# pangenome/gfasort

Hardware: AMD Instinct MI355X
Metric: SGD term-updates/sec, -p Y, 1M-node synthetic GFA (higher is better)
Workload: dtype f64

## Files before the change

gfasort_amd/build.py:

```python
import os
import subprocess
import sys

HERE = os.path.dirname(os.path.abspath(__file__))
CSRC = os.path.join(HERE, "csrc")
LIBDIR = os.path.join(HERE, "lib")
LIB = os.path.join(LIBDIR, "libgfasort_hip.so")
SOURCES = ["sgd_kernels_1d.hip", "sgd_kernels_1d_phased.hip", "sgd_kernels_nd.hip", "sgd_kernels_nd_team.hip", "sgd_kernels_nd_team_wide.hip", "index_kernels.hip",
           "capi.hip", "multi.hip"]
HEADERS = ["sgd_device.h", "sgd_kernel_common.h", "sgd_1d.h", "sgd_nd_team.h", "sgd_host.h", os.path.join("..", "..", "include", "gfasort_hip.h")]

HIPCC_FLAGS = ["--offload-arch=gfx950", "-O3", "-std=c++17", "-fPIC",
               "-ffp-contract=off", "-munsafe-fp-atomics", "-Wall", "-Wno-unused-function"]
OBJDIR = os.path.join(HERE, "lib", "obj")


def _stale():
    if not os.path.exists(LIB):
        return True
    t = os.path.getmtime(LIB)
    deps = [os.path.join(CSRC, s) for s in SOURCES + HEADERS] + [os.path.abspath(__file__)]
    return any(os.path.getmtime(d) > t for d in deps)


def build_hip(force=False, verbose=False):
    if not force and not _stale():
        return LIB
    os.makedirs(OBJDIR, exist_ok=True)
    hipcc = os.environ.get("HIPCC", "/opt/rocm/bin/hipcc")
    hdr_t = max(os.path.getmtime(os.path.join(CSRC, h)) for h in HEADERS)

    def compile_one(src):
        obj = os.path.join(OBJDIR, src.replace(".hip", ".o"))
        sp = os.path.join(CSRC, src)
        if not force and os.path.exists(obj) and os.path.getmtime(obj) > max(os.path.getmtime(sp), hdr_t):
            return obj
        cmd = [hipcc] + HIPCC_FLAGS + ["-c", "-o", obj, sp]
        if verbose:
            print(" ".join(cmd), file=sys.stderr)
        subprocess.check_call(cmd)
        return obj

    from concurrent.futures import ThreadPoolExecutor
# ... 48 lines not shown
```

gfasort_amd/csrc/sgd_1d.h:

```cpp
#pragma once
#include "sgd_kernel_common.h"

namespace gfs {

struct RefTerm1D { uint32_t i, j; int crowd; double term_dist; };

template <bool LDS_TABLES>
__device__ __forceinline__ bool ref_sample_1d(const KArgs &a, const uint4 *path_tab, const double *zeta_tab, Rng &rng,
                                              const uint64_t step_idx, const uint4 &ra, RefTerm1D &t) {
    uint4 rb; uint64_t sa, sb; uint32_t cnt, path;
    if (!sample_pair_from<LDS_TABLES>(a, path_tab, zeta_tab, rng, step_idx, ra, rb, sa, sb, cnt, path)) return false;
    t.term_dist = fabs(rec_pos(ra) - rec_pos(rb));
    if (t.term_dist == 0.0) return false;
    t.crowd = crowd_shift<false>(a, ra, rb);
    t.i = ra.x; t.j = rb.x;
    return t.i != 0xFFFFFFFFu && t.j != 0xFFFFFFFFu;
}

template <bool LDS_TABLES, bool ATOMIC_LOADS, bool TRACE>
__device__ __forceinline__ void ref_run_1d(const KArgs &a, const uint4 *path_tab, const double *zeta_tab, Rng &rng,
                                           const uint32_t quota, const uint64_t max_att, const uint32_t tid,
                                           uint32_t &done, uint32_t &att, uint32_t &ntr) {
    double *x = a.x;
    uint32_t d = 0; uint64_t t = 0;
// ... 5 lines not shown
        RefTerm1D cur;
        if (!ref_sample_1d<LDS_TABLES>(a, path_tab, zeta_tab, rng, s_a, r_a, cur)) continue;
        const double mu = crowd_scale(fmin(a.it.eta * (1.0 / cur.term_dist), 1.0), cur.crowd);
        double dx;
        if (a.dbg & 2u) dx = (double)cur.i - (double)cur.j;
        else dx = load_pos<ATOMIC_LOADS>(x + cur.i) - load_pos<ATOMIC_LOADS>(x + cur.j);
        if (dx == 0.0) dx = 1e-9;
        const double mag = fabs(dx);
        const double delta = mu * (mag - cur.term_dist) / 2.0;
        const double r = delta / mag;
        const double r_x = r * dx;
        if (d + 1u < quota && t < max_att) { s_a = sample_step(a, rng); r_a = a.step_rec[s_a]; drawn = true; }
        if (a.dbg & 1u) { asm volatile("" :: "v"(r_x)); }
        else {
            add_pos(x + cur.i, -r_x);
            add_pos(x + cur.j, r_x);
        }
        ++d;
        if (TRACE) record_trace(a, tid, ntr, cur.i, cur.j, cur.term_dist);
    }
    done += d;
    att += t > 0xFFFFFFFFull ? 0xFFFFFFFFu : (uint32_t)t;
}

struct TeamState {
    Rng rng;
    Leader L = {0, 0, 0, 0, 0, 0, 0, 0};
    uint32_t left = 0, cool = 0, colour = 0, seg = 0;
    uint32_t p = 0;
    uint32_t done = 0, att = 0, ntr = 0;
};

struct Trip {
    uint64_t sa = 0, sb = 0;
    uint4 ra = make_uint4(0, 0, 0, 0), rb = make_uint4(0, 0, 0, 0);
    uint4 rc = make_uint4(0, 0, 0, 0);
    bool twin = false;
    bool valid = false;
    int mshift = 0;
    bool two = false;
    bool fused = false;
    uint32_t k = 1;
    uint32_t off = 0;
};

template <int B>
__device__ __forceinline__ void expand_trip(const KArgs &a, const Leader &L, int t, uint32_t seg, uint32_t p, uint32_t colour, int sub, int q, Trip &tr) {
    constexpr int RUNS = 64 / B;
    const int ll = t * RUNS + q;
    const uint32_t okw = bcast<B>(L.ok, ll), cnt = bcast<B>(L.cnt, ll);
    const uint32_t ok = leader_ok(okw, p);
    const uint32_t ra0 = p ? bcast<B>(L.ra1, ll) : bcast<B>(L.ra0, ll), rb0 = p ? bcast<B>(L.rb1, ll) : bcast<B>(L.rb0, ll);
    const uint64_t first = bcast_first<B>(L, ll);
    tr.k = (B == 64 && ((okw | (okw >> 8)) & 1u) && cnt >= 2u * B) ? run_trips(a.chain, (uint32_t)B, cnt) : 1u;
    tr.off = B == 64 ? run_offset((uint32_t)B, cnt, tr.k, ra0, rb0, seg) : 0u;
    tr.mshift = merged_trip_shift<B>(ok, cnt, ra0, rb0, tr.off);
    const bool two = !(a.dbg & 0x08u) && two_colour<B>(ok, cnt, ra0, rb0);
    tr.two = B == 64 ? two : (__any(two) != 0);
    tr.ra = make_uint4(0, 0, 0, 0); tr.rb = make_uint4(0, 0, 0, 0); tr.rc = make_uint4(0, 0, 0, 0);
    tr.fused = B == 64 && tr.mshift != 0 && colour == 0 && two && !(a.dbg & 0x100u);
    tr.twin = B == 64 && p == 0u && a.partners == 2u && (okw & 3u) == 3u && ((okw >> 8) & 3u) == 3u && !(a.dbg & 0x04u);
    const uint32_t rb1 = bcast<B>(L.rb1, ll);
    if (tr.twin) {
        const int64_t gap = (int64_t)rb0 - (int64_t)rb1, lim = 192;
        if (gap < lim && gap > -lim) tr.twin = false;
    }
    if (tr.twin) {
        tr.sa = first + ra0 + tr.off + (uint32_t)sub;
        tr.sb = first + rb0 + tr.off + (((uint32_t)sub + ((okw >> 2) & 7u)) & 63u);
        const uint64_t sc = first + rb1 + tr.off + (((uint32_t)sub + ((okw >> 10) & 7u)) & 63u);
        tr.valid = true;
        tr.ra = a.step_rec[tr.sa]; tr.rb = a.step_rec[tr.sb]; tr.rc = a.step_rec[sc];
        return;
    }
    if (tr.fused) {
        const int dst = sub + tr.mshift;
        tr.sa = first + merged_trip_base(cnt, ra0, tr.off) + (uint32_t)sub;
        tr.sb = (uint64_t)((int64_t)tr.sa + tr.mshift);
        tr.valid = dst < 0 || dst > 63;
        tr.ra = a.step_rec[tr.sa];
        tr.rb = a.step_rec[tr.sb];
        return;
    }
    tr.valid = expand_run<B>(ok, first, cnt, ra0, rb0, sub, colour, tr.off, tr.sa, tr.sb);
    if (tr.valid) { tr.ra = a.step_rec[tr.sa]; tr.rb = a.step_rec[tr.sb]; }
}

__device__ __forceinline__ double term_move(const KArgs &a, double term_dist, double xi, double xj, int crowd) {
    double mu = crowd_scale(fmin(a.it.eta * (1.0 / term_dist), 1.0), crowd);
    double dx = xi - xj;
    if (dx == 0.0) dx = 1e-9;
    double mag = fabs(dx);
    double delta = mu * (mag - term_dist) / 2.0;
    double r = delta / mag;
    return r * dx;
}

__device__ __forceinline__ double shfl_f64(double v, int src) { return __shfl(v, src, 64); }

template <bool ATOMIC_LOADS, bool TRACE>
__device__ __forceinline__ bool fused_trip(const KArgs &a, TeamState &ts, const Trip &cur, const int lane,
                                           const uint32_t tid, const uint64_t wave_quota, uint64_t &wave_done) {
    double *x = a.x;
    const int s = cur.mshift, z = s < 0 ? -s : s;
    const int dst = lane + s, src = lane - s;
    const bool out = cur.valid;
    const int dstc = out ? lane : dst, srcc = (src < 0 || src > 63) ? lane : src;
    const uint32_t grp = ((cur.off + (uint32_t)lane) / (uint32_t)z) & 1u;
    const uint32_t node = cur.ra.x, pnode = cur.rb.x;
    double xo = 0.0, xp = 0.0;
    if (!(a.dbg & 2u)) {
        if (node != 0xFFFFFFFFu) xo = load_pos<ATOMIC_LOADS>(x + node);
        if (out && pnode != 0xFFFFFFFFu) xp = load_pos<ATOMIC_LOADS>(x + pnode);
    } else { xo = (double)node; xp = (double)pnode; }
    const double term_dist = fabs(rec_pos(cur.ra) - rec_pos(cur.rb));
    const int crowd = crowd_shift<true>(a, cur.ra, cur.rb);
    const bool term_ok = term_dist != 0.0 && node != 0xFFFFFFFFu && pnode != 0xFFFFFFFFu;
    double acc = 0.0;
    bool touched = false, second = true;
#pragma unroll
    for (uint32_t colour = 0; colour < 2u; ++colour) {
        ++ts.att;
        const bool valid = quota_cut(term_ok && grp == colour, lane, wave_quota, wave_done);
        const double xpart_in = shfl_f64(xo, dstc);
        const double xj = out ? xp : xpart_in;
        double r_x = 0.0;
        if (valid) {
            r_x = term_move(a, term_dist, xo, xj, crowd);
            ++ts.done;
            if (TRACE) record_trace(a, tid, ts.ntr, node, pnode, term_dist);
        }
        const double rv = shfl_f64(r_x, srcc);
        const int vsrc = __shfl((int)valid, srcc, 64);
        const bool recv = src >= 0 && src <= 63 && vsrc != 0;
        if (valid) xo = xo - r_x;
        if (recv) xo = xo + rv;
        if (valid) { acc = touched ? acc - r_x : -r_x; touched = true; }
        if (recv) { acc = touched ? acc + rv : rv; touched = true; }
        if (valid && out && !(a.dbg & 1u)) add_pos(x + pnode, r_x);
        if (colour == 0 && wave_done >= wave_quota) { second = false; break; }
    }
    if (touched && !(a.dbg & 1u)) add_pos(x + node, acc);
    return second;
}

template <bool ATOMIC_LOADS, bool TRACE>
__device__ __forceinline__ bool twin_trip(const KArgs &a, TeamState &ts, const Trip &cur, const int lane,
                                          const uint32_t tid, const uint64_t wave_quota, uint64_t &wave_done) {
    double *x = a.x;
    const uint32_t node = cur.ra.x, nb = cur.rb.x, nc = cur.rc.x;
    double xa = 0.0, xb = 0.0, xc = 0.0;
    if (!(a.dbg & 2u)) {
        if (node != 0xFFFFFFFFu) xa = load_pos<ATOMIC_LOADS>(x + node);
        if (nb != 0xFFFFFFFFu) xb = load_pos<ATOMIC_LOADS>(x + nb);
        if (nc != 0xFFFFFFFFu) xc = load_pos<ATOMIC_LOADS>(x + nc);
    } else { xa = (double)node; xb = (double)nb; xc = (double)nc; }
    const double pa = rec_pos(cur.ra);
    double acc = 0.0;
    bool touched = false, second = true;
#pragma unroll
    for (uint32_t p = 0; p < 2u; ++p) {
        ++ts.att;
        const uint4 &rp = p ? cur.rc : cur.rb;
        const uint32_t pn = p ? nc : nb;
        const double term_dist = fabs(pa - rec_pos(rp));
        const bool valid = quota_cut(term_dist != 0.0 && node != 0xFFFFFFFFu && pn != 0xFFFFFFFFu,
                                     lane, wave_quota, wave_done);
        if (valid) {
            const double r_x = term_move(a, term_dist, xa, p ? xc : xb, crowd_shift<true>(a, cur.ra, rp));
            ++ts.done;
            if (TRACE) record_trace(a, tid, ts.ntr, node, pn, term_dist);
            xa = xa - r_x;
            acc = touched ? acc - r_x : -r_x; touched = true;
            if (!(a.dbg & 1u)) add_pos(x + pn, r_x);
        }
        if (p == 0u && wave_done >= wave_quota) { second = false; break; }
    }
    if (touched && !(a.dbg & 1u)) add_pos(x + node, acc);
    return second;
}

template <int B, bool LDS_TABLES, bool ATOMIC_LOADS, bool TRACE>
__device__ __forceinline__ void team_iteration(const KArgs &a, const uint4 *path_tab, const double *zeta_tab,
                                               TeamState &ts, const uint32_t tid, const uint64_t wave_quota, const IterConsts *itp = nullptr) {
    const int lane = threadIdx.x & 63;
    const int sub = lane & (B - 1);
    const int q = lane / B;
    const uint64_t max_passes = (uint64_t)a.attempt_factor * (wave_quota / (64u * B) + 1u) + 16u;
    uint64_t wave_done = 0, passes = 0;
    double *x = a.x;
    while (wave_done < wave_quota && passes < max_passes) {
        if (ts.left == 0 || ts.cool != (uint32_t)a.it.cooling) {
            ++passes;
            KArgs as;
            reload_kargs(as);
            if (itp) {
                const IterConsts *ip = itp;
                asm volatile("" : "+s"(ip));
                as.it = *ip;
            }
            ts.L = sample_leader<LDS_TABLES>(as, path_tab, zeta_tab, ts.rng);
            ts.left = B; ts.cool = (uint32_t)a.it.cooling; ts.colour = 0; ts.seg = 0; ts.p = 0;
        }
        const Leader &L = ts.L;
        int t = B - (int)ts.left;
        uint32_t colour = ts.colour, seg = ts.seg, p = ts.p;
        Trip cur;
        expand_trip<B>(a, L, t, seg, p, colour, sub, q, cur);
        for (;;) {
            int t_n = t; uint32_t colour_n = 0u, seg_n = seg, p_n = p;
            if (colour == 0 && cur.two && !cur.fused) colour_n = 1u;
            else if (p == 0u && a.partners == 2u && !cur.twin) p_n = 1u;
            else if (seg + 1u < cur.k) { seg_n = seg + 1u; p_n = 0u; }
            else { t_n = t + 1; seg_n = 0u; p_n = 0u; }
            const bool have_n = t_n < B;
            Trip nxt;
            if (have_n) expand_trip<B>(a, L, t_n, seg_n, p_n, colour_n, sub, q, nxt);
            if (B == 64 && cur.twin) {
                if (!twin_trip<ATOMIC_LOADS, TRACE>(a, ts, cur, lane, tid, wave_quota, wave_done)) {
                    ts.colour = 0u; ts.seg = seg; ts.p = 1u;
                    break;
                }
                ts.colour = 0u; ts.seg = seg_n; ts.p = 0u;
                if (t_n != t) --ts.left;
                if (wave_done >= wave_quota || !have_n) break;
                cur = nxt; t = t_n; colour = colour_n; seg = seg_n; p = p_n;
                continue;
            }
            if (B == 64 && cur.fused) {
                if (!fused_trip<ATOMIC_LOADS, TRACE>(a, ts, cur, lane, tid, wave_quota, wave_done)) {
                    ts.colour = 1u; ts.seg = seg; ts.p = p;
                    break;
                }
                ts.colour = 0u; ts.seg = seg_n; ts.p = p_n;
                if (t_n != t) --ts.left;
                if (wave_done >= wave_quota || !have_n) break;
                cur = nxt; t = t_n; colour = colour_n; seg = seg_n; p = p_n;
                continue;
            }
            ++ts.att;
            ts.colour = colour_n; ts.seg = seg_n; ts.p = p_n;
            if (t_n != t) --ts.left;
            bool valid = cur.valid;
            const uint4 ra = cur.ra, rb = cur.rb;
            const int mshift = cur.mshift;
            double term_dist = 0.0;
            uint32_t i = 0, j = 0;
            if (valid) {
                term_dist = fabs(rec_pos(ra) - rec_pos(rb));
                i = ra.x; j = rb.x;
                valid = term_dist != 0.0 && i != 0xFFFFFFFFu && j != 0xFFFFFFFFu;
            }
            valid = quota_cut(valid, lane, wave_quota, wave_done);
            double xi = 0.0, xj = 0.0;
            if (valid) {
                if (a.dbg & 2u) { xi = (double)i; xj = (double)j; }
                else { xi = load_pos<ATOMIC_LOADS>(x + i); xj = load_pos<ATOMIC_LOADS>(x + j); }
            }
            double r_x = 0.0;
            if (valid) {
                r_x = term_move(a, term_dist, xi, xj, crowd_shift<true>(a, ra, rb));
                ++ts.done;
                if (TRACE) record_trace(a, tid, ts.ntr, i, j, term_dist);
            }
            bool o1f = valid, o2f = valid; uint32_t o1s = i, o2s = j; double o1v = -r_x, o2v = r_x;
            if (B == 64 && mshift != 0) {
                const int z = mshift < 0 ? -mshift : mshift;
                const int src = lane - mshift;
                const int srcc = src < 0 ? 0 : (src > 63 ? 63 : src);
                const double rv = __shfl(r_x, srcc, 64);
                const uint32_t js = (uint32_t)__shfl((int)j, srcc, 64);
                const int vs = __shfl((int)valid, srcc, 64);
                const bool resting = (((cur.off + (uint32_t)lane) / (uint32_t)z) & 1u) != colour;
                if (resting && src >= 0 && src < 64 && vs) { o1f = true; o1s = js; o1v = rv; }
                const int dst = lane + mshift;
                o2f = valid && (dst < 0 || dst > 63);
            }
            if (!(a.dbg & 1u)) {
                if (o1f) add_pos(x + o1s, o1v);
                if (o2f) add_pos(x + o2s, o2v);
            }
            if (wave_done >= wave_quota) break;
            if (!have_n) break;
            cur = nxt; t = t_n; colour = colour_n; seg = seg_n; p = p_n;
        }
    }
// ... 4 lines not shown
```

gfasort_amd/csrc/sgd_device.h:

```cpp
#pragma once
#include <hip/hip_runtime.h>
#include <stdint.h>

namespace gfs {

__device__ __forceinline__ int32_t sat_i32(double v) {
    if (v != v) return 0;
    if (v <= -2147483648.0) return INT32_MIN;
    if (v >= 2147483647.0) return INT32_MAX;
    return (int32_t)v;
}

__device__ __forceinline__ double fpp_split(double a, int32_t e, double fb) {
    int32_t high = (int32_t)((uint64_t)__double_as_longlong(a) >> 32);
    int32_t diff = (int32_t)((uint32_t)high - 1072632447u);
    int32_t new_high = sat_i32(fb * (double)diff + 1072632447.0);
    double frac = __longlong_as_double((long long)(((uint64_t)(uint32_t)new_high) << 32));
    double base = a, r = 1.0;
    int32_t ex = e;
    while (ex != 0) {
        if (ex & 1) r *= base;
        base *= base;
        ex >>= 1;
    }
    return r * frac;
}

struct Rng {
    uint64_t s0, s1, s2, s3;
    __device__ __forceinline__ uint64_t next() {
        uint64_t result = s0 + s3;
        uint64_t t = s1 << 17;
        s2 ^= s0; s3 ^= s1; s1 ^= s2; s0 ^= s3;
        s2 ^= t;
        s3 = (s3 << 45) | (s3 >> 19);
// ... 121 lines not shown
        if (back || fwd) {
            uint32_t room = back ? rank_a : (cnt - rank_a - 1u);
            uint32_t jump = a.space < room ? a.space : room;
            double zeta = zeta_tab[space_index(a, jump)];
            uint32_t z = dirty_zipf(a.it, jump, zeta, rng.f64());
            if (back) rank_b = rank_a >= z ? rank_a - z : 0u;
            else { uint64_t t = (uint64_t)rank_a + z; rank_b = t < cnt - 1u ? (uint32_t)t : cnt - 1u; }
        }
    } else {
        rank_b = rng.uniform32(cnt, pr.z);
    }
    if (rank_a == rank_b) return false;
    sa = step_idx;
    sb = first + rank_b;
    rb = a.step_rec[sb];
    cnt_out = cnt; path_out = path;
    return true;
}
template <bool LDS_TABLES>
__device__ __forceinline__ bool sample_pair(const KArgs &a, const uint4 *path_tab, const double *zeta_tab,
                                            Rng &rng, uint4 &ra, uint4 &rb, uint64_t &sa, uint64_t &sb,
                                            uint32_t &cnt_out, uint32_t &path_out) {
    const uint64_t step_idx = sample_step(a, rng);
    ra = a.step_rec[step_idx];
    return sample_pair_from<LDS_TABLES>(a, path_tab, zeta_tab, rng, step_idx, ra, rb, sa, sb, cnt_out, path_out);
}

struct Leader {
    uint32_t first_lo, first_hi, cnt;
    uint32_t ra0, rb0;
    uint32_t ok;
    uint32_t ra1, rb1;
};
__device__ __forceinline__ uint32_t leader_ok(uint32_t okw, uint32_t p) { return (p ? okw >> 8 : okw) & 0x1Fu; }

constexpr uint32_t TEAM_CHUNK = 2048;
constexpr uint32_t ND_TEAM_CHUNK = 4096;

__device__ __forceinline__ uint32_t run_trips(uint32_t chain, uint32_t bundle, uint32_t cnt) {
    const uint32_t room = cnt / (4u * bundle);
    if (room < 2u || chain < 2u) return 1u;
    const uint32_t p2 = 1u << (31 - __clz((int)room));
    return p2 < chain ? p2 : chain;
}
__device__ __forceinline__ uint32_t run_offset(uint32_t bundle, uint32_t cnt, uint32_t k, uint32_t ra0, uint32_t rb0, uint32_t seg) {
    const uint32_t z = ra0 < rb0 ? rb0 - ra0 : ra0 - rb0;
    return seg * (z < bundle ? cnt / k : bundle);
}

__device__ __forceinline__ uint32_t draw_partner(const KArgs &a, const double *zeta_tab, Rng &rng, const uint32_t cnt,
                                                 const uint32_t thresh, const uint32_t slot0, uint32_t &ra, uint32_t &rb) {
    rb = ra;
    if (a.it.cooling || rng.flip() == 1u) {
        bool back = false, fwd = false;
        if (ra > 0u && (rng.flip() == 1u || ra == cnt - 1u)) back = true;
        else if (ra < cnt - 1u) fwd = true;
        if (back || fwd) {
            uint32_t room = back ? ra : (cnt - ra - 1u);
            uint32_t jump = a.space < room ? a.space : room;
            double zeta = zeta_tab[space_index(a, jump)];
            uint32_t z = dirty_zipf(a.it, jump, zeta, rng.f64());
            if (back) rb = ra >= z ? ra - z : 0u;
            else { uint64_t t = (uint64_t)ra + z; rb = t < cnt - 1u ? (uint32_t)t : cnt - 1u; }
        }
    } else {
        rb = rng.uniform32(cnt, thresh);
    }
    uint32_t ok = (rb != ra) ? 1u : 0u;
    if (ok && cnt >= 2u * a.bundle && slot0 != 0xFFFFFFFFu && !(a.dbg & 0x10u)) {
        const int64_t jump = (int64_t)rb - (int64_t)ra;
        const int64_t Bn = (int64_t)a.bundle;
        const int64_t Rn = Bn * (int64_t)run_trips(a.chain, a.bundle, cnt);
        if (jump >= Bn + 8 || jump <= -(Bn + 8)) {
            const int64_t A = a.bundle < 8u ? (int64_t)a.bundle : 8;
            const uint32_t sh = slot0 & (uint32_t)(A - 1);
            if (ra >= sh) {
                const int64_t na = (int64_t)ra - (int64_t)sh;
                const int64_t r = ((jump % A) + A) % A, zp = jump - r, nb = na + zp;
                if (!(a.dbg & 0x20u) && na + Rn <= (int64_t)cnt && nb >= 0 && nb + Rn <= (int64_t)cnt && (zp >= Bn || zp <= -Bn)) {
                    ra = (uint32_t)na; rb = (uint32_t)nb; ok = 1u | 2u | ((uint32_t)r << 2);
                } else if (rb >= sh) { ra -= sh; rb -= sh; }
            }
        }
    }
    return ok;
}

template <bool LDS_TABLES>
__device__ __forceinline__ Leader sample_leader(const KArgs &a, const uint4 *path_tab, const double *zeta_tab, Rng &rng) {
    Leader L;
    const uint64_t s0 = sample_step(a, rng);
    const uint4 r0 = a.step_rec[s0];
    const uint4 pr = path_tab[rec_path(r0)];
    L.first_lo = pr.x; L.first_hi = pr.w; L.cnt = pr.y;
    L.ra0 = (uint32_t)(s0 - path_first(pr)); L.rb0 = L.ra0;
    L.ra1 = L.ra0; L.rb1 = L.ra0;
    L.ok = 0;
    if (L.cnt == 1u) return L;
    L.ok = draw_partner(a, zeta_tab, rng, L.cnt, pr.z, r0.x, L.ra0, L.rb0);
    if (a.partners == 2u) L.ok |= draw_partner(a, zeta_tab, rng, L.cnt, pr.z, r0.x, L.ra1, L.rb1) << 8;
    return L;
}

template <int B>
__device__ __forceinline__ bool two_colour(uint32_t ok, uint32_t cnt, uint32_t ra0, uint32_t rb0) {
    if ((ok & 3u) != 1u || cnt < 2u * B) return false;
    const int64_t s = (int64_t)rb0 - (int64_t)ra0;
    return s < (int64_t)B && s > -(int64_t)B;
}

template <int B>
__device__ __forceinline__ bool expand_run(uint32_t ok, uint64_t first, uint32_t cnt, uint32_t ra0, uint32_t rb0,
                                           int sub, uint32_t colour, uint32_t off, uint64_t &sa, uint64_t &sb) {
    if (!(ok & 1u)) return false;
    if (ok & 2u) {
        if (colour) return false;
        sa = first + ra0 + off + (uint32_t)sub;
        sb = first + rb0 + off + (((uint32_t)sub + ((ok >> 2) & 7u)) & (uint32_t)(B - 1));
        return true;
    }
    uint32_t ra_l = ra0, rb_l = rb0;
    const uint32_t l = off + (uint32_t)sub;
    if (l != 0 || colour) {
        if (cnt < 2u * B) return false;
        const int64_t shift = (int64_t)rb0 - (int64_t)ra0;
        const uint32_t z = (uint32_t)(shift < 0 ? -shift : shift);
        if (z < (uint32_t)B) { if (((l / z) & 1u) != colour) return false; }
        else if (colour) return false;
        uint64_t ra_w = (uint64_t)ra0 + l;
        if (ra_w >= cnt) ra_w -= cnt;
        if (ra_w >= cnt) ra_w -= cnt;
        ra_l = (uint32_t)ra_w;
        int64_t t = (int64_t)ra_l + shift;
        if (t < 0 || t > (int64_t)cnt - 1) {
            if (z < (uint32_t)B) return false;
            t = (int64_t)ra_l - shift;
            if (t < 0 || t > (int64_t)cnt - 1) return false;
        }
        rb_l = (uint32_t)t;
    }
    sa = first + ra_l;
    sb = first + rb_l;
    return true;
}

__device__ __forceinline__ double rec_pos(const uint4 &r) {
    return (double)rec_pos_u64(r);
}

}
```

gfasort_amd/csrc/sgd_kernel_common.h:

```cpp
#pragma once
#include "sgd_device.h"

namespace gfs {

struct TraceTerm { uint32_t i, j; double d; };

template <bool ATOMIC_LOADS>
__device__ __forceinline__ double load_pos(const double *p) {
    if (ATOMIC_LOADS)
        return __hip_atomic_load(p, __ATOMIC_RELAXED, __HIP_MEMORY_SCOPE_AGENT);
    return *p;
}
__device__ __forceinline__ void add_pos(double *p, double v) {
    (void)__hip_atomic_fetch_add(p, v, __ATOMIC_RELAXED, __HIP_MEMORY_SCOPE_AGENT);
}

template <bool LDS_TABLES>
__device__ __forceinline__ void stage_tables(const KArgs &a, unsigned char *smem,
                                             const uint4 *&path_tab, const double *&zeta_tab) {
    if (LDS_TABLES) {
        uint4 *lp = reinterpret_cast<uint4 *>(smem);
        double *lz = reinterpret_cast<double *>(smem + (size_t)a.n_paths * sizeof(uint4));
        for (uint32_t k = threadIdx.x; k < a.n_paths; k += blockDim.x) lp[k] = a.path_rec[k];
        for (uint32_t k = threadIdx.x; k < a.zlen_staged; k += blockDim.x) lz[k] = a.zetas[k];
// ... 80 lines not shown
    return (uint32_t)__shfl((int)v, leader_lane, 64);
}


template <int B>
__device__ __forceinline__ uint64_t bcast_first(const Leader &L, int leader_lane) {
    return ((uint64_t)bcast<B>(L.first_hi, leader_lane) << 32) | bcast<B>(L.first_lo, leader_lane);
}

template <class State>
__device__ __forceinline__ void load_pass(const KArgs &a, uint32_t tid, State &ts, uint32_t &flips) {
    if (!a.lead) return;
    const uint64_t T = a.n_streams;
    ts.L.first_lo = a.lead[tid]; ts.L.first_hi = a.lead[T + tid]; ts.L.cnt = a.lead[2 * T + tid];
    ts.L.ra0 = a.lead[3 * T + tid]; ts.L.rb0 = a.lead[4 * T + tid];
    const uint32_t w = a.lead[5 * T + tid];
    ts.L.ra1 = a.lead[6 * T + tid]; ts.L.rb1 = a.lead[7 * T + tid];
    ts.L.ok = (w & 0x1Fu) | ((w >> 27) << 8);
    flips = (w >> 5) & 7u;
    const uint32_t ws = (uint32_t)__builtin_amdgcn_readfirstlane((int)w);
    ts.left = (ws >> 8) & 0xFFu; ts.cool = (ws >> 16) & 1u; ts.colour = (ws >> 17) & 1u; ts.seg = (ws >> 18) & 0xFFu; ts.p = (ws >> 26) & 1u;
}
template <class State>
__device__ __forceinline__ void store_pass(const KArgs &a, uint32_t tid, const State &ts, const uint32_t flips) {
    if (!a.lead) return;
    const uint64_t T = a.n_streams;
    a.lead[tid] = ts.L.first_lo; a.lead[T + tid] = ts.L.first_hi; a.lead[2 * T + tid] = ts.L.cnt;
    a.lead[3 * T + tid] = ts.L.ra0; a.lead[4 * T + tid] = ts.L.rb0;
    a.lead[5 * T + tid] = (ts.L.ok & 0x1Fu) | ((flips & 7u) << 5) | (ts.left << 8) | (ts.cool << 16) | (ts.colour << 17) | (ts.seg << 18) |
                          (ts.p << 26) | (((ts.L.ok >> 8) & 0x1Fu) << 27);
    a.lead[6 * T + tid] = ts.L.ra1; a.lead[7 * T + tid] = ts.L.rb1;
}

template <int B>
__device__ __forceinline__ int merged_trip_shift(uint32_t ok, uint32_t cnt, uint32_t ra0, uint32_t rb0, uint32_t off) {
    if (B != 64 || (ok & 3u) != 1u || cnt < 128u) return 0;
    const int64_t s = (int64_t)rb0 - (int64_t)ra0;
    if (s == 0 || s >= 64 || s <= -64) return 0;
    uint64_t base = (uint64_t)ra0 + (uint64_t)off;
    if (base >= cnt) base -= cnt;
    if (base + 64u > cnt) return 0;
    if (s > 0 ? base + 63u + (uint64_t)s > (uint64_t)cnt - 1u : (int64_t)base + s < 0) return 0;
    return (int)s;
}
__device__ __forceinline__ uint32_t merged_trip_base(uint32_t cnt, uint32_t ra0, uint32_t off) {
    uint64_t base = (uint64_t)ra0 + (uint64_t)off;
    if (base >= cnt) base -= cnt;
    return (uint32_t)base;
}

constexpr uint32_t POOL_SLOTS = 16, POOL_STRIDE = 16;
__host__ __device__ __forceinline__ uint32_t pool_slots(uint32_t n_waves) {
    const uint32_t s = n_waves / 16u;
    return s < 1u ? 1u : (s > POOL_SLOTS ? POOL_SLOTS : s);
}

struct PoolShare { uint32_t slot, cap; };
__device__ __forceinline__ PoolShare pool_share(const KArgs &a, const uint32_t wave, const uint32_t n_waves) {
    const uint32_t slots = pool_slots(n_waves), slot = wave % slots;
    const uint64_t total = (uint64_t)a.quota_base * a.n_streams + a.quota_rem;
    return {slot, (uint32_t)(total / slots + (slot < total % slots ? 1u : 0u))};
}
__device__ __forceinline__ PoolShare pool_share_single(const KArgs &a) {
    return {0u, (uint32_t)((uint64_t)a.quota_base * a.n_streams + a.quota_rem)};
}

__device__ __forceinline__ void send_claim(uint32_t *pool_counter, const uint32_t chunk, uint32_t &claim) {
    if ((threadIdx.x & 63u) == 0) claim = __hip_atomic_fetch_add(pool_counter, chunk, __ATOMIC_RELAXED, __HIP_MEMORY_SCOPE_AGENT);
}

template <class ChunkOf, class Body>
__device__ __forceinline__ void pool_walk(KArgs &a, const IterConsts *its, const uint32_t n_iters, uint32_t *pool, const PoolShare ps,
                                          ChunkOf &&chunk_of, Body &&body) {
    uint32_t k = 0, claim = 0;
    a.it = its[0];
    uint32_t chunk = chunk_of();
    send_claim(pool + ps.slot * POOL_STRIDE, chunk, claim);
    while (k < n_iters) {
        const uint32_t old = (uint32_t)__builtin_amdgcn_readfirstlane((int)claim);
        if (old >= ps.cap) {
            if (++k == n_iters) break;
            a.it = its[k];
// ... 27 lines not shown
```

Baseline: 104.5 billion.

## Hoist per-slot trip planning out of per-trip expansion and add fast quota path

Leader-slot fields (k, short jumps, twin flag, ok bits) are now computed once per slot into a packed SlotPlan instead of being re-broadcast and recomputed for every trip expansion. Step addresses are split into a wave-uniform base plus a small per-lane offset, which may let the compiler use scalar base addressing. A cheaper quota_cut_1d counts valid lanes with a ballot popcount when the remaining wave quota is at least 64. The shared helpers move into a host/device header with a host selftest that checks equivalence against the old logic. The cost is extra live registers for the plan, which could lower occupancy.

```diff
diff --git a/gfasort_amd/build.py b/gfasort_amd/build.py
--- a/gfasort_amd/build.py
+++ b/gfasort_amd/build.py
@@ -8,7 +8,7 @@
 LIB = os.path.join(LIBDIR, "libgfasort_hip.so")
 SOURCES = ["sgd_kernels_1d.hip", "sgd_kernels_1d_phased.hip", "sgd_kernels_nd.hip", "sgd_kernels_nd_team.hip", "sgd_kernels_nd_team_wide.hip", "index_kernels.hip",
            "capi.hip", "multi.hip"]
-HEADERS = ["sgd_device.h", "sgd_kernel_common.h", "sgd_1d.h", "sgd_nd_team.h", "sgd_host.h", os.path.join("..", "..", "include", "gfasort_hip.h")]
+HEADERS = ["sgd_device.h", "sgd_trip_plan.h", "sgd_kernel_common.h", "sgd_1d.h", "sgd_nd_team.h", "sgd_host.h", os.path.join("..", "..", "include", "gfasort_hip.h")]
 
 HIPCC_FLAGS = ["--offload-arch=gfx950", "-O3", "-std=c++17", "-fPIC",
                "-ffp-contract=off", "-munsafe-fp-atomics", "-Wall", "-Wno-unused-function"]
diff --git a/gfasort_amd/csrc/host/trip_plan_selftest.cpp b/gfasort_amd/csrc/host/trip_plan_selftest.cpp
--- /dev/null
+++ b/gfasort_amd/csrc/host/trip_plan_selftest.cpp
@@ -0,0 +1,126 @@
+#include <cinttypes>
+#include <cstdio>
+#include <cstdlib>
+#include <vector>
+#include "../sgd_trip_plan.h"
+
+using namespace gfs;
+
+static unsigned long long n_plans = 0, n_trips = 0, n_lanes = 0;
+
+#define CHECK(cond)                                                                                                           \
+    do {                                                                                                                      \
+        if (!(cond)) {                                                                                                        \
+            std::printf("DIFF %s (line %d): cnt %u chain %u okw 0x%x ra0 %u rb0 %u ra1 %u rb1 %u seg %u p %u colour %u sub %d dbg 0x%x partners %u\n", \
+                        #cond, __LINE__, cnt, chain, okw, ra0, rb0, ra1, rb1, seg, p, colour, sub, dbg, partners);            \
+            std::exit(1);                                                                                                     \
+        }                                                                                                                     \
+    } while (0)
+
+template <int B>
+static void sweep_leader(uint32_t chain, uint32_t partners, uint32_t dbg, uint64_t first, uint32_t cnt, uint32_t okw,
+                         uint32_t ra0, uint32_t rb0, uint32_t ra1, uint32_t rb1, uint32_t meta_rep, bool deep, int lane_step) {
+    uint32_t seg = 0, p = 0, colour = 0; int sub = 0;
+    const SlotPlan pl = make_plan<B>(chain, partners, dbg, first, cnt, okw, ra0, rb0, ra1, rb1);
+    ++n_plans;
+    const uint32_t k_old = (B == 64 && ((okw | (okw >> 8)) & 1u) && cnt >= 2u * B) ? run_trips(chain, (uint32_t)B, cnt) : 1u;
+    CHECK(pl.k() == k_old && pl.okw() == okw && pl.first == first && pl.cnt == cnt && pl.spread == cnt / k_old);
+    bool twin_old = B == 64 && partners == 2u && (okw & 3u) == 3u && ((okw >> 8) & 3u) == 3u && !(dbg & 0x04u);
+    if (twin_old) { const int64_t gap = (int64_t)rb0 - (int64_t)rb1, lim = 192; if (gap < lim && gap > -lim) twin_old = false; }
+    CHECK(pl.twin() == twin_old);
+    if (!deep) { CHECK(pl.meta == meta_rep); return; }
+    for (seg = 0; seg < k_old; ++seg) for (p = 0; p < partners; ++p) for (colour = 0; colour < 2u; ++colour) {
+        const uint32_t ok = leader_ok(okw, p), ra = p ? ra1 : ra0, rb = p ? rb1 : rb0;
+        const uint32_t off_old = B == 64 ? run_offset((uint32_t)B, cnt, k_old, ra, rb, seg) : 0u;
+        const int mshift_old = merged_trip_shift<B>(ok, cnt, ra, rb, off_old);
+        const bool two_old = !(dbg & 0x08u) && two_colour<B>(ok, cnt, ra, rb);
+        const bool fused_old = B == 64 && mshift_old != 0 && colour == 0 && two_old && !(dbg & 0x100u);
+        const bool twin_trip_old = p == 0u && twin_old;
+        if (colour == 1u && !two_old) continue;
+        const TripShape s = plan_trip<B>(pl, dbg, seg, p, colour);
+        ++n_trips;
+        CHECK(s.off == off_old);
+        CHECK(s.mshift == mshift_old && s.two == two_old && s.fused == fused_old && s.twin == twin_trip_old);
+        if (mshift_old != 0) CHECK(s.base == merged_trip_base(cnt, ra, off_old));
+        for (sub = 0; sub < B; sub += lane_step) {
+            LaneSteps ls;
+            const bool loads = trip_lane_steps<B>(pl, s, p, colour, sub, ls);
+            ++n_lanes;
+            if (twin_trip_old) {
+                CHECK(loads && ls.base_a + ls.la == first + ra0 + off_old + (uint32_t)sub);
+                CHECK(ls.base_b + ls.lb == first + rb0 + off_old + (((uint32_t)sub + ((okw >> 2) & 7u)) & 63u));
+                CHECK(ls.base_c + ls.lc == first + rb1 + off_old + (((uint32_t)sub + ((okw >> 10) & 7u)) & 63u));
+            } else if (fused_old) {
+                const uint64_t sa = first + merged_trip_base(cnt, ra, off_old) + (uint32_t)sub;
+                CHECK(loads && ls.base_a + ls.la == sa && ls.base_b + ls.lb == (uint64_t)((int64_t)sa + mshift_old));
+            } else {
+                uint64_t sa = 0, sb = 0;
+                const bool valid = expand_run<B>(ok, first, cnt, ra, rb, sub, colour, off_old, sa, sb);
+                CHECK(loads == valid);
+                if (valid) CHECK(ls.base_a + ls.la == sa && ls.base_b + ls.lb == sb);
+            }
+        }
+    }
+}
+
+int main(int argc, char **argv) {
+    const uint32_t max_cnt = argc > 1 ? (uint32_t)std::strtoul(argv[1], nullptr, 10) : 5000u;
+    std::vector<uint32_t> cnts;
+    for (uint32_t c = 1; c <= max_cnt; ++c) cnts.push_back(c);
+    cnts.push_back(156250u);
+    const uint64_t first = 0x123456789ull;
+    for (const uint32_t cnt : cnts) {
+        const int64_t jumps[] = {0, 1, -1, 2, -2, 7, -7, 8, -8, 63, -63, 64, -64, 71, -71, 72, -72, 191, -191, 192, -192, 193, -193,
+                                 (int64_t)cnt - 1, -((int64_t)cnt - 1)};
+        const int nj = (int)(sizeof(jumps) / sizeof(jumps[0]));
+        const int lane_step = (cnt <= 300u || cnt % 64u < 2u || cnt > max_cnt) ? 1 : 21;
+        const uint32_t ras[3] = {0u, cnt / 2u, cnt - 1u};
+        for (int ia = 0; ia < 3; ++ia) for (int i = 0; i < nj; ++i) for (int order = 0; order < 2; ++order) {
+            const uint32_t a0 = ras[ia];
+            const int64_t j0 = jumps[order ? (i + 5) % nj : i], j1 = jumps[order ? i : (i + 5) % nj];
+            uint32_t ra[2] = {a0, a0}, rb[2] = {a0, a0}, okp[2] = {0u, 0u};
+            const int64_t jj[2] = {j0, j1};
+            uint32_t k_path = run_trips(64u, 64u, cnt);
+            for (int q = 0; q < 2; ++q) {
+                const int64_t b = (int64_t)a0 + jj[q];
+                if (jj[q] == 0 || b < 0 || b > (int64_t)cnt - 1) continue;
+                rb[q] = (uint32_t)b; okp[q] = 1u;
+            }
+            for (int aligned = 0; aligned < 2; ++aligned) {
+                uint32_t ra_v[2] = {ra[0], ra[1]}, rb_v[2] = {rb[0], rb[1]}, ok_v[2] = {okp[0], okp[1]};
+                if (aligned) {
+                    bool any = false;
+                    for (int q = 0; q < 2; ++q) {
+                        const int64_t jump = jj[q], Rn = 64 * (int64_t)k_path;
+                        if (!okp[q] || (jump < 72 && jump > -72)) continue;
+                        const uint32_t sh = (uint32_t)(i & 7);
+                        if (a0 < sh) continue;
+                        const int64_t na = (int64_t)a0 - sh, r = ((jump % 8) + 8) % 8, zp = jump - r, nb = na + zp;
+                        if (na + Rn <= (int64_t)cnt && nb >= 0 && nb + Rn <= (int64_t)cnt && (zp >= 64 || zp <= -64)) {
+                            ra_v[q] = (uint32_t)na; rb_v[q] = (uint32_t)nb; ok_v[q] = 1u | 2u | ((uint32_t)r << 2); any = true;
+                        }
+                    }
+                    if (!any) continue;
+                }
+                const uint32_t okw = ok_v[0] | (ok_v[1] << 8);
+                uint32_t last_k = 0, meta_rep = 0;
+                for (uint32_t chain = 1; chain <= 64u; ++chain) {
+                    const uint32_t k = run_trips(chain, 64u, cnt);
+                    const bool deep = k != last_k;
+                    if (deep) meta_rep = make_plan<64>(chain, 2u, 0u, first, cnt, okw, ra_v[0], rb_v[0], ra_v[1], rb_v[1]).meta;
+                    last_k = k;
+                    sweep_leader<64>(chain, 2u, 0u, first, cnt, okw, ra_v[0], rb_v[0], ra_v[1], rb_v[1], meta_rep, deep, (chain & (chain - 1u)) ? 21 : lane_step);
+                }
+                sweep_leader<64>(16u, 1u, 0u, first, cnt, okw & 0x1Fu, ra_v[0], rb_v[0], ra_v[0], ra_v[0], 0u, true, lane_step);
+                if (i % 4 == 0) {
+                    sweep_leader<64>(16u, 2u, 0x04u, first, cnt, okw, ra_v[0], rb_v[0], ra_v[1], rb_v[1], 0u, true, 9);
+                    sweep_leader<64>(16u, 2u, 0x08u, first, cnt, okw, ra_v[0], rb_v[0], ra_v[1], rb_v[1], 0u, true, 9);
+                    sweep_leader<64>(16u, 2u, 0x100u, first, cnt, okw, ra_v[0], rb_v[0], ra_v[1], rb_v[1], 0u, true, 9);
+                    if (!aligned) sweep_leader<16>(16u, 1u, 0u, first, cnt, okw & 0x1Fu, ra_v[0], rb_v[0], ra_v[0], ra_v[0], 0u, true, 3);
+                }
+            }
+        }
+    }
+    std::printf("ok %llu %llu %llu\n", n_plans, n_trips, n_lanes);
+    return 0;
+}
diff --git a/gfasort_amd/csrc/sgd_1d.h b/gfasort_amd/csrc/sgd_1d.h
--- a/gfasort_amd/csrc/sgd_1d.h
+++ b/gfasort_amd/csrc/sgd_1d.h
@@ -61,7 +61,6 @@
 };
 
 struct Trip {
-    uint64_t sa = 0, sb = 0;
     uint4 ra = make_uint4(0, 0, 0, 0), rb = make_uint4(0, 0, 0, 0);
     uint4 rc = make_uint4(0, 0, 0, 0);
     bool twin = false;
@@ -69,50 +68,37 @@
     int mshift = 0;
     bool two = false;
     bool fused = false;
-    uint32_t k = 1;
     uint32_t off = 0;
 };
 
 template <int B>
-__device__ __forceinline__ void expand_trip(const KArgs &a, const Leader &L, int t, uint32_t seg, uint32_t p, uint32_t colour, int sub, int q, Trip &tr) {
+__device__ __forceinline__ SlotPlan slot_plan(const KArgs &a, const Leader &L, int t, int q) {
     constexpr int RUNS = 64 / B;
     const int ll = t * RUNS + q;
-    const uint32_t okw = bcast<B>(L.ok, ll), cnt = bcast<B>(L.cnt, ll);
-    const uint32_t ok = leader_ok(okw, p);
-    const uint32_t ra0 = p ? bcast<B>(L.ra1, ll) : bcast<B>(L.ra0, ll), rb0 = p ? bcast<B>(L.rb1, ll) : bcast<B>(L.rb0, ll);
-    const uint64_t first = bcast_first<B>(L, ll);
-    tr.k = (B == 64 && ((okw | (okw >> 8)) & 1u) && cnt >= 2u * B) ? run_trips(a.chain, (uint32_t)B, cnt) : 1u;
-    tr.off = B == 64 ? run_offset((uint32_t)B, cnt, tr.k, ra0, rb0, seg) : 0u;
-    tr.mshift = merged_trip_shift<B>(ok, cnt, ra0, rb0, tr.off);
-    const bool two = !(a.dbg & 0x08u) && two_colour<B>(ok, cnt, ra0, rb0);
-    tr.two = B == 64 ? two : (__any(two) != 0);
+    return make_plan<B>(a.chain, a.partners, a.dbg, bcast_first<B>(L, ll), bcast<B>(L.cnt, ll), bcast<B>(L.ok, ll),
+                        bcast<B>(L.ra0, ll), bcast<B>(L.rb0, ll), bcast<B>(L.ra1, ll), bcast<B>(L.rb1, ll));
+}
+
+template <int B>
+__device__ __forceinline__ void expand_trip(const KArgs &a, const SlotPlan &pl, uint32_t seg, uint32_t p, uint32_t colour, int sub, Trip &tr) {
+    const TripShape s = plan_trip<B>(pl, a.dbg, seg, p, colour);
+    tr.off = s.off; tr.mshift = s.mshift; tr.fused = s.fused; tr.twin = s.twin;
+    tr.two = B == 64 ? s.two : (__any(s.two) != 0);
     tr.ra = make_uint4(0, 0, 0, 0); tr.rb = make_uint4(0, 0, 0, 0); tr.rc = make_uint4(0, 0, 0, 0);
-    tr.fused = B == 64 && tr.mshift != 0 && colour == 0 && two && !(a.dbg & 0x100u);
-    tr.twin = B == 64 && p == 0u && a.partners == 2u && (okw & 3u) == 3u && ((okw >> 8) & 3u) == 3u && !(a.dbg & 0x04u);
-    const uint32_t rb1 = bcast<B>(L.rb1, ll);
-    if (tr.twin) {
-        const int64_t gap = (int64_t)rb0 - (int64_t)rb1, lim = 192;
-        if (gap < lim && gap > -lim) tr.twin = false;
-    }
-    if (tr.twin) {
-        tr.sa = first + ra0 + tr.off + (uint32_t)sub;
-        tr.sb = first + rb0 + tr.off + (((uint32_t)sub + ((okw >> 2) & 7u)) & 63u);
-        const uint64_t sc = first + rb1 + tr.off + (((uint32_t)sub + ((okw >> 10) & 7u)) & 63u);
-        tr.valid = true;
-        tr.ra = a.step_rec[tr.sa]; tr.rb = a.step_rec[tr.sb]; tr.rc = a.step_rec[sc];
-        return;
-    }
-    if (tr.fused) {
-        const int dst = sub + tr.mshift;
-        tr.sa = first + merged_trip_base(cnt, ra0, tr.off) + (uint32_t)sub;
-        tr.sb = (uint64_t)((int64_t)tr.sa + tr.mshift);
-        tr.valid = dst < 0 || dst > 63;
-        tr.ra = a.step_rec[tr.sa];
-        tr.rb = a.step_rec[tr.sb];
-        return;
-    }
-    tr.valid = expand_run<B>(ok, first, cnt, ra0, rb0, sub, colour, tr.off, tr.sa, tr.sb);
-    if (tr.valid) { tr.ra = a.step_rec[tr.sa]; tr.rb = a.step_rec[tr.sb]; }
+    LaneSteps ls;
+    const bool loads = trip_lane_steps<B>(pl, s, p, colour, sub, ls);
+    tr.valid = loads;
+    if (s.fused) { const int dst = sub + s.mshift; tr.valid = dst < 0 || dst > 63; }
+    if (loads) { tr.ra = (a.step_rec + ls.base_a)[ls.la]; tr.rb = (a.step_rec + ls.base_b)[ls.lb]; }
+    if (B == 64 && s.twin) tr.rc = (a.step_rec + ls.base_c)[ls.lc];
+}
+
+__device__ __forceinline__ bool quota_cut_1d(bool valid, const int lane, const uint64_t wave_quota, uint64_t &wave_done) {
+    if (wave_quota - wave_done >= 64u) {
+        wave_done += (uint32_t)__popcll(__ballot(valid));
+        return valid;
+    }
+    return quota_cut(valid, lane, wave_quota, wave_done);
 }
 
 __device__ __forceinline__ double term_move(const KArgs &a, double term_dist, double xi, double xj, int crowd) {
@@ -150,7 +136,7 @@
 #pragma unroll
     for (uint32_t colour = 0; colour < 2u; ++colour) {
         ++ts.att;
-        const bool valid = quota_cut(term_ok && grp == colour, lane, wave_quota, wave_done);
+        const bool valid = quota_cut_1d(term_ok && grp == colour, lane, wave_quota, wave_done);
         const double xpart_in = shfl_f64(xo, dstc);
         const double xj = out ? xp : xpart_in;
         double r_x = 0.0;
@@ -193,7 +179,7 @@
         const uint4 &rp = p ? cur.rc : cur.rb;
         const uint32_t pn = p ? nc : nb;
         const double term_dist = fabs(pa - rec_pos(rp));
-        const bool valid = quota_cut(term_dist != 0.0 && node != 0xFFFFFFFFu && pn != 0xFFFFFFFFu,
+        const bool valid = quota_cut_1d(term_dist != 0.0 && node != 0xFFFFFFFFu && pn != 0xFFFFFFFFu,
                                      lane, wave_quota, wave_done);
         if (valid) {
             const double r_x = term_move(a, term_dist, xa, p ? xc : xb, crowd_shift<true>(a, cur.ra, rp));
@@ -234,17 +220,22 @@
         const Leader &L = ts.L;
         int t = B - (int)ts.left;
         uint32_t colour = ts.colour, seg = ts.seg, p = ts.p;
+        SlotPlan plan = slot_plan<B>(a, L, t, q);
+        uint32_t k = plan.k();
         Trip cur;
-        expand_trip<B>(a, L, t, seg, p, colour, sub, q, cur);
+        expand_trip<B>(a, plan, seg, p, colour, sub, cur);
         for (;;) {
             int t_n = t; uint32_t colour_n = 0u, seg_n = seg, p_n = p;
             if (colour == 0 && cur.two && !cur.fused) colour_n = 1u;
             else if (p == 0u && a.partners == 2u && !cur.twin) p_n = 1u;
-            else if (seg + 1u < cur.k) { seg_n = seg + 1u; p_n = 0u; }
+            else if (seg + 1u < k) { seg_n = seg + 1u; p_n = 0u; }
             else { t_n = t + 1; seg_n = 0u; p_n = 0u; }
             const bool have_n = t_n < B;
             Trip nxt;
-            if (have_n) expand_trip<B>(a, L, t_n, seg_n, p_n, colour_n, sub, q, nxt);
+            if (have_n) {
+                if (t_n != t) { plan = slot_plan<B>(a, L, t_n, q); k = plan.k(); }
+                expand_trip<B>(a, plan, seg_n, p_n, colour_n, sub, nxt);
+            }
             if (B == 64 && cur.twin) {
                 if (!twin_trip<ATOMIC_LOADS, TRACE>(a, ts, cur, lane, tid, wave_quota, wave_done)) {
                     ts.colour = 0u; ts.seg = seg; ts.p = 1u;
@@ -280,7 +271,7 @@
                 i = ra.x; j = rb.x;
                 valid = term_dist != 0.0 && i != 0xFFFFFFFFu && j != 0xFFFFFFFFu;
             }
-            valid = quota_cut(valid, lane, wave_quota, wave_done);
+            valid = quota_cut_1d(valid, lane, wave_quota, wave_done);
             double xi = 0.0, xj = 0.0;
             if (valid) {
                 if (a.dbg & 2u) { xi = (double)i; xj = (double)j; }
diff --git a/gfasort_amd/csrc/sgd_device.h b/gfasort_amd/csrc/sgd_device.h
--- a/gfasort_amd/csrc/sgd_device.h
+++ b/gfasort_amd/csrc/sgd_device.h
@@ -1,6 +1,7 @@
 #pragma once
 #include <hip/hip_runtime.h>
 #include <stdint.h>
+#include "sgd_trip_plan.h"
 
 namespace gfs {
 
@@ -188,21 +189,10 @@
     uint32_t ok;
     uint32_t ra1, rb1;
 };
-__device__ __forceinline__ uint32_t leader_ok(uint32_t okw, uint32_t p) { return (p ? okw >> 8 : okw) & 0x1Fu; }
 
 constexpr uint32_t TEAM_CHUNK = 2048;
 constexpr uint32_t ND_TEAM_CHUNK = 4096;
 
-__device__ __forceinline__ uint32_t run_trips(uint32_t chain, uint32_t bundle, uint32_t cnt) {
-    const uint32_t room = cnt / (4u * bundle);
-    if (room < 2u || chain < 2u) return 1u;
-    const uint32_t p2 = 1u << (31 - __clz((int)room));
-    return p2 < chain ? p2 : chain;
-}
-__device__ __forceinline__ uint32_t run_offset(uint32_t bundle, uint32_t cnt, uint32_t k, uint32_t ra0, uint32_t rb0, uint32_t seg) {
-    const uint32_t z = ra0 < rb0 ? rb0 - ra0 : ra0 - rb0;
-    return seg * (z < bundle ? cnt / k : bundle);
-}
 
 __device__ __forceinline__ uint32_t draw_partner(const KArgs &a, const double *zeta_tab, Rng &rng, const uint32_t cnt,
                                                  const uint32_t thresh, const uint32_t slot0, uint32_t &ra, uint32_t &rb) {
@@ -258,48 +248,6 @@
     return L;
 }
 
-template <int B>
-__device__ __forceinline__ bool two_colour(uint32_t ok, uint32_t cnt, uint32_t ra0, uint32_t rb0) {
-    if ((ok & 3u) != 1u || cnt < 2u * B) return false;
-    const int64_t s = (int64_t)rb0 - (int64_t)ra0;
-    return s < (int64_t)B && s > -(int64_t)B;
-}
-
-template <int B>
-__device__ __forceinline__ bool expand_run(uint32_t ok, uint64_t first, uint32_t cnt, uint32_t ra0, uint32_t rb0,
-                                           int sub, uint32_t colour, uint32_t off, uint64_t &sa, uint64_t &sb) {
-    if (!(ok & 1u)) return false;
-    if (ok & 2u) {
-        if (colour) return false;
-        sa = first + ra0 + off + (uint32_t)sub;
-        sb = first + rb0 + off + (((uint32_t)sub + ((ok >> 2) & 7u)) & (uint32_t)(B - 1));
-        return true;
-    }
-    uint32_t ra_l = ra0, rb_l = rb0;
-    const uint32_t l = off + (uint32_t)sub;
-    if (l != 0 || colour) {
-        if (cnt < 2u * B) return false;
-        const int64_t shift = (int64_t)rb0 - (int64_t)ra0;
-        const uint32_t z = (uint32_t)(shift < 0 ? -shift : shift);
-        if (z < (uint32_t)B) { if (((l / z) & 1u) != colour) return false; }
-        else if (colour) return false;
-        uint64_t ra_w = (uint64_t)ra0 + l;
-        if (ra_w >= cnt) ra_w -= cnt;
-        if (ra_w >= cnt) ra_w -= cnt;
-        ra_l = (uint32_t)ra_w;
-        int64_t t = (int64_t)ra_l + shift;
-        if (t < 0 || t > (int64_t)cnt - 1) {
-            if (z < (uint32_t)B) return false;
-            t = (int64_t)ra_l - shift;
-            if (t < 0 || t > (int64_t)cnt - 1) return false;
-        }
-        rb_l = (uint32_t)t;
-    }
-    sa = first + ra_l;
-    sb = first + rb_l;
-    return true;
-}
-
 __device__ __forceinline__ double rec_pos(const uint4 &r) {
     return (double)rec_pos_u64(r);
 }
diff --git a/gfasort_amd/csrc/sgd_kernel_common.h b/gfasort_amd/csrc/sgd_kernel_common.h
--- a/gfasort_amd/csrc/sgd_kernel_common.h
+++ b/gfasort_amd/csrc/sgd_kernel_common.h
@@ -136,22 +136,6 @@
     a.lead[6 * T + tid] = ts.L.ra1; a.lead[7 * T + tid] = ts.L.rb1;
 }
 
-template <int B>
-__device__ __forceinline__ int merged_trip_shift(uint32_t ok, uint32_t cnt, uint32_t ra0, uint32_t rb0, uint32_t off) {
-    if (B != 64 || (ok & 3u) != 1u || cnt < 128u) return 0;
-    const int64_t s = (int64_t)rb0 - (int64_t)ra0;
-    if (s == 0 || s >= 64 || s <= -64) return 0;
-    uint64_t base = (uint64_t)ra0 + (uint64_t)off;
-    if (base >= cnt) base -= cnt;
-    if (base + 64u > cnt) return 0;
-    if (s > 0 ? base + 63u + (uint64_t)s > (uint64_t)cnt - 1u : (int64_t)base + s < 0) return 0;
-    return (int)s;
-}
-__device__ __forceinline__ uint32_t merged_trip_base(uint32_t cnt, uint32_t ra0, uint32_t off) {
-    uint64_t base = (uint64_t)ra0 + (uint64_t)off;
-    if (base >= cnt) base -= cnt;
-    return (uint32_t)base;
-}
 
 constexpr uint32_t POOL_SLOTS = 16, POOL_STRIDE = 16;
 __host__ __device__ __forceinline__ uint32_t pool_slots(uint32_t n_waves) {
diff --git a/gfasort_amd/csrc/sgd_trip_plan.h b/gfasort_amd/csrc/sgd_trip_plan.h
--- /dev/null
+++ b/gfasort_amd/csrc/sgd_trip_plan.h
@@ -0,0 +1,191 @@
+#pragma once
+#include <stdint.h>
+
+#if defined(__HIPCC__)
+#define GFS_HD __host__ __device__ __forceinline__
+#else
+#define GFS_HD inline
+#endif
+
+namespace gfs {
+
+GFS_HD int clz32(uint32_t v) {
+#if defined(__HIP_DEVICE_COMPILE__)
+    return __clz((int)v);
+#else
+    return __builtin_clz(v);
+#endif
+}
+
+GFS_HD uint32_t leader_ok(uint32_t okw, uint32_t p) { return (p ? okw >> 8 : okw) & 0x1Fu; }
+
+GFS_HD uint32_t run_trips(uint32_t chain, uint32_t bundle, uint32_t cnt) {
+    const uint32_t room = cnt / (4u * bundle);
+    if (room < 2u || chain < 2u) return 1u;
+    const uint32_t p2 = 1u << (31 - clz32(room));
+    return p2 < chain ? p2 : chain;
+}
+GFS_HD uint32_t run_offset(uint32_t bundle, uint32_t cnt, uint32_t k, uint32_t ra0, uint32_t rb0, uint32_t seg) {
+    const uint32_t z = ra0 < rb0 ? rb0 - ra0 : ra0 - rb0;
+    return seg * (z < bundle ? cnt / k : bundle);
+}
+
+template <int B>
+GFS_HD bool two_colour(uint32_t ok, uint32_t cnt, uint32_t ra0, uint32_t rb0) {
+    if ((ok & 3u) != 1u || cnt < 2u * B) return false;
+    const int64_t s = (int64_t)rb0 - (int64_t)ra0;
+    return s < (int64_t)B && s > -(int64_t)B;
+}
+
+template <int B>
+GFS_HD bool expand_run(uint32_t ok, uint64_t first, uint32_t cnt, uint32_t ra0, uint32_t rb0,
+                       int sub, uint32_t colour, uint32_t off, uint64_t &sa, uint64_t &sb) {
+    if (!(ok & 1u)) return false;
+    if (ok & 2u) {
+        if (colour) return false;
+        sa = first + ra0 + off + (uint32_t)sub;
+        sb = first + rb0 + off + (((uint32_t)sub + ((ok >> 2) & 7u)) & (uint32_t)(B - 1));
+        return true;
+    }
+    uint32_t ra_l = ra0, rb_l = rb0;
+    const uint32_t l = off + (uint32_t)sub;
+    if (l != 0 || colour) {
+        if (cnt < 2u * B) return false;
+        const int64_t shift = (int64_t)rb0 - (int64_t)ra0;
+        const uint32_t z = (uint32_t)(shift < 0 ? -shift : shift);
+        if (z < (uint32_t)B) { if (((l / z) & 1u) != colour) return false; }
+        else if (colour) return false;
+        uint64_t ra_w = (uint64_t)ra0 + l;
+        if (ra_w >= cnt) ra_w -= cnt;
+        if (ra_w >= cnt) ra_w -= cnt;
+        ra_l = (uint32_t)ra_w;
+        int64_t t = (int64_t)ra_l + shift;
+        if (t < 0 || t > (int64_t)cnt - 1) {
+            if (z < (uint32_t)B) return false;
+            t = (int64_t)ra_l - shift;
+            if (t < 0 || t > (int64_t)cnt - 1) return false;
+        }
+        rb_l = (uint32_t)t;
+    }
+    sa = first + ra_l;
+    sb = first + rb_l;
+    return true;
+}
+
+template <int B>
+GFS_HD int merged_trip_shift(uint32_t ok, uint32_t cnt, uint32_t ra0, uint32_t rb0, uint32_t off) {
+    if (B != 64 || (ok & 3u) != 1u || cnt < 128u) return 0;
+    const int64_t s = (int64_t)rb0 - (int64_t)ra0;
+    if (s == 0 || s >= 64 || s <= -64) return 0;
+    uint64_t base = (uint64_t)ra0 + (uint64_t)off;
+    if (base >= cnt) base -= cnt;
+    if (base + 64u > cnt) return 0;
+    if (s > 0 ? base + 63u + (uint64_t)s > (uint64_t)cnt - 1u : (int64_t)base + s < 0) return 0;
+    return (int)s;
+}
+GFS_HD uint32_t merged_trip_base(uint32_t cnt, uint32_t ra0, uint32_t off) {
+    uint64_t base = (uint64_t)ra0 + (uint64_t)off;
+    if (base >= cnt) base -= cnt;
+    return (uint32_t)base;
+}
+
+constexpr int64_t TWIN_GAP = 192;
+
+struct SlotPlan {
+    uint64_t first;
+    uint32_t cnt;
+    uint32_t ra0, rb0, ra1, rb1;
+    uint32_t spread;
+    uint32_t meta;
+    GFS_HD uint32_t ok(uint32_t p) const { return (p ? meta >> 5 : meta) & 0x1Fu; }
+    GFS_HD uint32_t okw() const { return (meta & 0x1Fu) | (((meta >> 5) & 0x1Fu) << 8); }
+    GFS_HD int sj(uint32_t p) const { return (int)(meta << (p ? 8 : 15)) >> 25; }
+    GFS_HD uint32_t k() const { return (meta >> 24) & 0x7Fu; }
+    GFS_HD bool twin() const { return (meta >> 31) != 0u; }
+    template <int B>
+    GFS_HD uint32_t stride(uint32_t p) const {
+        if (B != 64) return 0u;
+        return (sj(p) != 0 || !(ok(p) & 1u)) ? spread : (uint32_t)B;
+    }
+};
+
+template <int B>
+GFS_HD int short_jump(uint32_t ok, uint32_t cnt, uint32_t ra, uint32_t rb) {
+    if ((ok & 3u) != 1u || cnt < 2u * B) return 0;
+    const int64_t s = (int64_t)rb - (int64_t)ra;
+    return s < (int64_t)B && s > -(int64_t)B ? (int)s : 0;
+}
+
+template <int B>
+GFS_HD SlotPlan make_plan(uint32_t chain, uint32_t partners, uint32_t dbg, uint64_t first, uint32_t cnt, uint32_t okw,
+                          uint32_t ra0, uint32_t rb0, uint32_t ra1, uint32_t rb1) {
+    static_assert(B <= 64, "a short jump and K (<= 64: the seg field of a stored pass) are packed into 7 bits each");
+    SlotPlan pl;
+    pl.first = first; pl.cnt = cnt;
+    pl.ra0 = ra0; pl.rb0 = rb0; pl.ra1 = ra1; pl.rb1 = rb1;
+    const uint32_t k = (B == 64 && ((okw | (okw >> 8)) & 1u) && cnt >= 2u * B) ? run_trips(chain, (uint32_t)B, cnt) : 1u;
+    pl.spread = (k & (k - 1u)) == 0u ? cnt >> (31 - clz32(k)) : cnt / k;
+    const uint32_t sj0 = (uint32_t)short_jump<B>(leader_ok(okw, 0u), cnt, ra0, rb0) & 0x7Fu;
+    const uint32_t sj1 = (uint32_t)short_jump<B>(leader_ok(okw, 1u), cnt, ra1, rb1) & 0x7Fu;
+    const int64_t gap = (int64_t)rb0 - (int64_t)rb1;
+    const bool twin = B == 64 && partners == 2u && (okw & 3u) == 3u && ((okw >> 8) & 3u) == 3u && !(dbg & 0x04u) &&
+                      !(gap < TWIN_GAP && gap > -TWIN_GAP);
+    pl.meta = (okw & 0x1Fu) | (((okw >> 8) & 0x1Fu) << 5) | (sj0 << 10) | (sj1 << 17) | (k << 24) | ((twin ? 1u : 0u) << 31);
+    return pl;
+}
+
+struct TripShape {
+    uint32_t off;
+    uint32_t base;
+    int mshift;
+    bool two;
+    bool fused;
+    bool twin;
+};
+template <int B>
+GFS_HD TripShape plan_trip(const SlotPlan &pl, uint32_t dbg, uint32_t seg, uint32_t p, uint32_t colour) {
+    TripShape s;
+    const int sj = pl.sj(p);
+    s.off = seg * pl.template stride<B>(p);
+    uint64_t base = (uint64_t)(p ? pl.ra1 : pl.ra0) + (uint64_t)s.off;
+    if (base >= pl.cnt) base -= pl.cnt;
+    s.base = (uint32_t)base;
+    const bool inside = base + 64u <= pl.cnt &&
+                        (sj > 0 ? base + 63u + (uint64_t)sj <= (uint64_t)pl.cnt - 1u : (int64_t)base + sj >= 0);
+    s.mshift = (B == 64 && sj != 0 && inside) ? sj : 0;
+    s.two = sj != 0 && !(dbg & 0x08u);
+    s.fused = B == 64 && s.mshift != 0 && colour == 0u && s.two && !(dbg & 0x100u);
+    s.twin = p == 0u && pl.twin();
+    return s;
+}
+
+struct LaneSteps { uint64_t base_a, base_b, base_c; uint32_t la, lb, lc; };
+template <int B>
+GFS_HD bool trip_lane_steps(const SlotPlan &pl, const TripShape &s, uint32_t p, uint32_t colour, int sub, LaneSteps &ls) {
+    const uint32_t ok = pl.ok(p), ra = p ? pl.ra1 : pl.ra0, rb = p ? pl.rb1 : pl.rb0;
+    ls.base_c = pl.first; ls.lc = 0u;
+    if (s.twin) {
+        ls.base_a = pl.first + pl.ra0 + s.off; ls.la = (uint32_t)sub;
+        ls.base_b = pl.first + pl.rb0 + s.off; ls.lb = ((uint32_t)sub + ((pl.ok(0u) >> 2) & 7u)) & 63u;
+        ls.base_c = pl.first + pl.rb1 + s.off; ls.lc = ((uint32_t)sub + ((pl.ok(1u) >> 2) & 7u)) & 63u;
+        return true;
+    }
+    if (s.fused) {
+        ls.base_a = pl.first + s.base; ls.la = (uint32_t)sub;
+        ls.base_b = (uint64_t)((int64_t)ls.base_a + s.mshift); ls.lb = (uint32_t)sub;
+        return true;
+    }
+    if ((ok & 3u) == 3u) {
+        if (colour) return false;
+        ls.base_a = pl.first + ra + s.off; ls.la = (uint32_t)sub;
+        ls.base_b = pl.first + rb + s.off; ls.lb = ((uint32_t)sub + ((ok >> 2) & 7u)) & (uint32_t)(B - 1);
+        return true;
+    }
+    uint64_t qa = 0, qb = 0;
+    if (!expand_run<B>(ok, 0ull, pl.cnt, ra, rb, sub, colour, s.off, qa, qb)) return false;
+    ls.base_a = pl.first; ls.la = (uint32_t)qa;
+    ls.base_b = pl.first; ls.lb = (uint32_t)qb;
+    return true;
+}
+
+}
```

New measurement: 103.9 billion. No clear change (-0.6%).
